# cqf7419/LiDAR-GS

Hardware: AMD Instinct MI355X
Metric: LiDAR range-view frames/sec (fwd+bwd) (higher is better)
Workload: dtype f32

## Files before the change

__graft_entry__.py:

```python
import os
import sys

ROOT = os.path.dirname(os.path.abspath(__file__))
for _p in (ROOT, os.path.join(ROOT, "lidar-gs_amd"), os.path.join(ROOT, "tests")):
    if _p not in sys.path:
        sys.path.insert(0, _p)


def build():
    import build_hip
    so = build_hip.build()
    assert os.path.exists(so), so
    from oracle import lgo
    lgo.build()
    import diff_lidargs_rasterization
    import lidargs_optim
    print("built:", so)
    print("built:", build_hip.OPTIM_OUT)


def smoke():
    import numpy as np
    import torch
    assert torch.cuda.is_available(), "smoke() needs a HIP device"
    import build_hip
    build_hip.build()
    import lidargs_scenes as sc
    from util import GRAD_KEYS_SR, hip_forward_backward, oracle_forward_backward, parity
    P, H, W, seed = 4000, 16, 512, 1
    scene = sc.make_scene("shell", P, H, seed, random_view=True)
    grads = sc.upstream_grads(H, W, seed)
    hip = hip_forward_backward(scene, W, H, grads, device="cuda:0")
    ref = oracle_forward_backward(scene, W, H, grads)
# ... 24 lines not shown
```

lidar-gs_amd/build_hip.py:

```python
import os
import subprocess
import sys
from concurrent.futures import ThreadPoolExecutor

HERE = os.path.dirname(os.path.abspath(__file__))
CSRC = os.path.join(HERE, "csrc")
OBJ = os.path.join(HERE, "build")
OUT = os.path.join(HERE, "diff_lidargs_rasterization", "liblidargs_hip.so")
COMMON = ["--offload-arch=gfx950", "-O3", "-std=c++17", "-fPIC", "-munsafe-fp-atomics", "-fno-gpu-rdc", "-Wall",
          "-Wno-unused-function", "-Wno-unused-value"]
SOURCES = {
    "api.hip": [],
    "preprocess.hip": ["-ffp-contract=off"],
    "binning.hip": [],
    "shard.hip": [],
    "render.hip": ["-fno-slp-vectorize"],
    "neural_gaussians.hip": [],
    "lidar_loss.hip": [],
    "chamfer.hip": ["-ffp-contract=off"],
    "surfel.hip": ["-ffp-contract=off", "-fno-slp-vectorize"],
    "anchor_growing.hip": ["-ffp-contract=off"],
    "knn.hip": ["-ffp-contract=off"],
    "metrics.hip": ["-ffp-contract=off"],
}
OPTIM_OUT = os.path.join(HERE, "lidargs_optim", "liblidargs_optim.so")
OPTIM_INCLUDE = os.path.join(HERE, "..", "include_optim")
OPTIM_SOURCES = {
    "adam.hip": ["-ffp-contract=off"],
}


def build_id():
    import hashlib
    h = hashlib.sha1()
    files = sorted(os.path.join(CSRC, f) for f in os.listdir(CSRC)) + sorted(
        os.path.join(HERE, "..", "include", f) for f in os.listdir(os.path.join(HERE, "..", "include"))) + sorted(
        os.path.join(OPTIM_INCLUDE, f) for f in os.listdir(OPTIM_INCLUDE)) + [os.path.abspath(__file__)]
    for f in files:
        h.update(os.path.basename(f).encode()); h.update(open(f, "rb").read())
    return h.hexdigest()[:12]


def box_id():
    try:
        import re
        out = subprocess.run(["rocm-smi", "--showuniqueid"], capture_output=True, text=True, timeout=20).stdout
        m = re.search(r"Unique ID:\s*(0x[0-9a-fA-F]+|\w+)", out)
        if m:
            return m.group(1)
    except Exception:
        pass
    return None


def _stale(out, deps):
    if not os.path.exists(out):
        return True
    t = os.path.getmtime(out)
    return any(os.path.getmtime(d) > t for d in deps)


def needs_build():
    return _stale(OUT, [os.path.join(CSRC, f) for f in os.listdir(CSRC) if f not in OPTIM_SOURCES]
                  + [os.path.join(HERE, "..", "include", "lidargs_rasterizer.h"), __file__])


def optim_needs_build():
    return _stale(OPTIM_OUT, [os.path.join(CSRC, f) for f in OPTIM_SOURCES]
                  + [os.path.join(OPTIM_INCLUDE, f) for f in os.listdir(OPTIM_INCLUDE)] + [__file__])


def build(force=False, verbose=False):
    if not force and not needs_build() and not optim_needs_build():
        return OUT
    import fcntl
    os.makedirs(OBJ, exist_ok=True)
    with open(os.path.join(OBJ, ".lock"), "w") as lock:
        fcntl.flock(lock, fcntl.LOCK_EX)
        try:
            if force or needs_build():
                _build_locked(SOURCES, OUT, verbose)
            if force or optim_needs_build():
                _build_locked(OPTIM_SOURCES, OPTIM_OUT, verbose)
            return OUT
        finally:
            fcntl.flock(lock, fcntl.LOCK_UN)


def _build_locked(sources, out, verbose):
    hipcc = os.environ.get("HIPCC", "/opt/rocm/bin/hipcc")
    extra_all = os.environ.get("LIDARGS_EXTRA_HIPCC_FLAGS", "").split()

    def compile_one(item):
        src, extra = item
        obj = os.path.join(OBJ, src.replace(".hip", ".o"))
        cmd = [hipcc] + COMMON + extra + extra_all + ["-c", os.path.join(CSRC, src), "-o", obj]
        if verbose:
            print(" ".join(cmd))
# ... 17 lines not shown
```

lidar-gs_amd/csrc/api.hip:

```cpp
#include "lidargs_common.h"
#include "../../include/lidargs_rasterizer.h"

#include <math.h>
#include <stdio.h>
#include <stdlib.h>
#include <string.h>
#include <limits>
#include <algorithm>
#include <mutex>

namespace {
using lg::SegPlan;

thread_local char g_err[512] = "";
thread_local long long g_counters[10] = {0, 0, 0, 0, 0, 0, 0, 0, -1, -1};
thread_local int g_counters_on = 0;
struct CounterPage {
    unsigned long long* dev = nullptr; unsigned long long* host = nullptr; hipEvent_t done = nullptr; int device = -1; bool pending = false;
    bool ready() {
        int d = -1;
        if (hipGetDevice(&d) != hipSuccess) return false;
        if (dev && d == device) return true;
        if (dev) { (void)hipFree(dev); dev = nullptr; }
        if (done) { (void)hipEventDestroy(done); done = nullptr; }
// ... 188 lines not shown
struct Profiler {
    static constexpr int MAX_CALLS = 256;
    struct Call { int n = 0; const char* names[LIDARGS_MAX_STAGES]; hipEvent_t ev[LIDARGS_MAX_STAGES + 1]; bool created = false; };
    bool enabled = false;
    int every = 1;
    int seen[2] = {0, 0};
    int ncalls = 0;
    Call* calls = nullptr;
    Call* cur = nullptr;
};
Profiler g_prof;
}

namespace lg {
int api_fail(int code, const char* msg) { return fail(code, "%s", msg); }
int api_check_launch(hipStream_t s, int debug, const char* what) { return check_launch(s, debug, what); }
int api_read_words_zero_behind(const uint32_t* dev, int n, uint32_t* out, void* zero, size_t zero_bytes, hipStream_t s) {
    hipError_t e = (hipError_t)read_words_begin(dev, n, s);
    if (e == hipSuccess && zero && zero_bytes) e = hipMemsetAsync(zero, 0, zero_bytes, s);
    return e == hipSuccess ? read_words_end(n, out) : (int)e;
}
bool prune_footprints() {
    static const bool on = [] { const char* e = getenv("LIDARGS_NO_PRUNE"); return !(e && atoi(e) != 0); }();
    return on;
}
int tile_rows() { return forced_tile_rows() ? forced_tile_rows() : 4; }

FrameLayout frame_layout(int num_rendered, int W, int H, int col_lo, int col_hi, FrameVariant variant) {
    const bool surfel = variant == FRAME_SURFEL, shell = variant == FRAME_SHELL;
    FrameLayout L;
// ... 285 lines not shown
    if (!geom_buffer || !binning_buffer || !image_buffer) return fail(LIDARGS_ERR_STATE, "backward: missing forward buffers%s");
    if (!means3D || !viewmatrix || !radii || !dL_dpix || !dL_dout_depth || !dL_dout_occ || !dL_dmean2D ||
        !dL_dopacity || !dL_dcolor || !dL_dmean3D || !dL_dscale || !dL_drot || (cov3D_precomp && !dL_dcov3D))
        return fail(LIDARGS_ERR_INVALID_ARGUMENT, "backward: NULL required pointer%s");

    lg::GeomView geom; lg::geom_carve(geom_buffer, (size_t)P, lg::GAUSS_BUFFERS, &geom);
    if (col_lo >= 0 && (col_lo % LG_TILE_W || col_hi <= col_lo || col_hi > width)) return fail(LIDARGS_ERR_INVALID_ARGUMENT, "backward: bad column wedge%s");
    const lg::FrameLayout L = lg::frame_layout(R, width, height, col_lo, col_hi, mode.is_shell ? lg::FRAME_SHELL : lg::FRAME_GAUSS);
    lg::BinView bin; L.bin_carve(binning_buffer, &bin);
    lg::ImgView img; lg::img_carve(image_buffer, width, height, lg::make_grid(width, height, 4).num_tiles(), &img);
    lg::prof_begin(stream, 1);

    lg::ZeroRows zr;
    zr.add(dL_dmean2D, 4); zr.add(dL_dconic, 4); zr.add(dL_dopacity, 1); zr.add(dL_dcolor, 2); zr.add(dL_ddepths, 1); zr.add(dL_dmean3D, 3);
    zr.add(dL_dsphere_means3D, 3); zr.add(dL_dbasis_u1, 3); zr.add(dL_dbasis_u2, 3); zr.add(dL_dcov3D, 6); zr.add(dL_dscale, 3); zr.add(dL_drot, 4);
    lg::launch_zero_touched(geom.touched, reinterpret_cast<float4*>(geom.gacc), 4, (size_t)P, geom.tlist, geom.tcount, zr, stream);
    lg::prof_mark("bwd_zero", stream);

    lg::RenderBwdArgs rb;
    rb.walk.cnt = nullptr;
    rb.grid = L.grid; rb.ranges = img.ranges; rb.point_list = bin.val_a; rb.rec = geom.rec; rb.rowspan = geom.rowspan;
    rb.coltab = img.coltab; rb.rowtab = img.rowtab; rb.bg = background; rb.final_T = img.final_T;
    rb.seg = bin.seg; rb.S = L.S; rb.seg_len = L.plan.seg_len;
    rb.alive = L.gated ? bin.alive : nullptr;
    rb.flags = L.flags ? bin.flags : nullptr; rb.R = L.Rp;
    rb.T_final_global = mode.T_final_global; rb.behind = mode.behind;
    rb.dL_dpix = dL_dpix; rb.dL_ddepth = dL_dout_depth; rb.dL_docc = dL_dout_occ; rb.gacc = geom.gacc;
    if (L.work_list) rb.walk = lg::work_list(bin);
    lg::launch_render_backward(rb, stream);
    LG_STAGE_CHECK("render backward");
    lg::prof_mark("render_bwd", stream);

    lg::GaussBwdArgs gb;
    gb.P = P; gb.scale_modifier = scale_modifier;
    gb.view = viewmatrix;
    gb.means3D = means3D; gb.scales = scales; gb.rotations = rotations; gb.cov3D_precomp = cov3D_precomp; gb.radii = radii;
    gb.gacc = geom.gacc; gb.tlist = geom.tlist; gb.tcount = geom.tcount;
    gb.dL_dmean2D = dL_dmean2D; gb.dL_dconic = dL_dconic; gb.dL_dopacity = dL_dopacity; gb.dL_dcolor = dL_dcolor;
    gb.dL_ddepths = dL_ddepths; gb.dL_dbasis_u1 = dL_dbasis_u1; gb.dL_dbasis_u2 = dL_dbasis_u2;
    gb.dL_dsphere = dL_dsphere_means3D; gb.dL_dmean3D = dL_dmean3D; gb.dL_dcov3D = dL_dcov3D; gb.dL_dscale = dL_dscale;
    gb.dL_drot = dL_drot;
    lg::launch_gaussian_backward(gb, stream);
    LG_STAGE_CHECK("gaussian backward");
// ... 448 lines not shown
```

lidar-gs_amd/csrc/lidargs_common.h:

```cpp
#pragma once
#include <hip/hip_runtime.h>
#include <stdint.h>
#include <stddef.h>

#define LG_TILE_W 16
#define LG_WAVE_ROWS 4
#define LG_CHANNELS 2

#define LG_SEG_TPASS 0
#define LG_SEG_C0 1
#define LG_SEG_C1 2
#define LG_SEG_D 3
#define LG_SEG_TEND 4
#define LG_SEG_TBREAK 5
#define LG_SEG_LAST 6
#define LG_SEG_PLANES 7

#define LG_REGION 256

namespace lg {

struct Carver {
    char* p;
    explicit Carver(char* base) : p(base) {}
// ... 238 lines not shown
    BufferWidths buf;
    size_t bin_carve(char* base, BinView* v) const { return lg::bin_carve(base, Rp, patches, grid.waves_per_tile, S, buf, v); }
};
FrameLayout frame_layout(int num_rendered, int W, int H, int col_lo, int col_hi, FrameVariant variant);

struct BinSpec {
    FrameVariant variant;
    int tile_rows;
    long long capacity;
    unsigned* status_host;
    const char* what;
};
struct BinnedFrame { FrameLayout L; BinView bin; size_t R; };
int bin_frame(const BinSpec& spec, const GeomView& geom, uint2* ranges, size_t P, int W, int H, int col_lo, int col_hi, bool compact,
              char* (*binning_alloc)(void*, size_t), void* binning_user, int debug, hipStream_t s, BinnedFrame* out);
struct ZeroRows { static constexpr int MAX = 12; float* p[MAX]; int w[MAX]; int n = 0;
                  void add(float* q, int width) { if (q && n < MAX) { p[n] = q; w[n] = width; n++; } } };
void launch_zero_touched(const uint8_t* touched, float4* acc, int line_f4, size_t P, uint8_t* tlist, uint16_t* tcount, const ZeroRows& zr, hipStream_t s);
void launch_touch_all(uint8_t* touched, const int* radii, size_t P, hipStream_t s);

void launch_setup_tables(const float* beams, int W, int H, ImgView img, hipStream_t s);
void launch_preprocess(const PreprocessParams& pp, const float* means3D, const float* scales, const float* rotations,
                       const float* opacities, const float* colors, const float* cov3D_precomp, const float* beams,
                       int* radii, int* radii_xy, GeomView g, const ImgView* tables, bool filter_only, hipStream_t s);
void launch_mark_visible(int P, const float* means3D, const float* view, unsigned char* present, hipStream_t s);
void launch_debug_rects(int n, int surfel, const float* p_cr, const int* r_xy, int gx, int gy, int* rects, hipStream_t s);

void launch_exclusive_scan(const uint32_t* in, uint32_t* out, size_t n, uint32_t* total_out, uint32_t* scratch, hipStream_t s);
struct RadixTail { const void* src = nullptr; void* dst = nullptr; int mode = 0; };
struct KeyBias { uint32_t kmin, cull; const uint32_t* lin_span = nullptr; };
struct RangeSortRest { KeyBias bias; int end_bit, max_bits; };
inline RangeSortRest range_sort_rest(uint32_t kinv, uint32_t kmax) {
    RangeSortRest r;
// ... 100 lines not shown

struct RenderBwdArgs {
    TileGrid grid;
    const uint2* ranges; const uint32_t* point_list; const float4* rec; const uint32_t* rowspan;
    const float2* coltab; const float2* rowtab;
    const float* bg;
    const float* final_T;
    const float* seg; int S; int seg_len;
    const uint8_t* flags; size_t R;
    const uint8_t* alive;
    const float* T_final_global;
    const float* behind;
    const float* dL_dpix; const float* dL_ddepth; const float* dL_docc;
    float* gacc;
    WorkList walk;
};
void launch_render_backward(const RenderBwdArgs& a, hipStream_t s);
void launch_count_backward_entries(const RenderBwdArgs& a, unsigned long long* out, hipStream_t s);
void note_forward(size_t P, size_t R, const FrameLayout& L, const uint32_t* totals, const uint8_t* flags, const uint8_t* touched,
                  const RenderBwdArgs* view, hipStream_t s);

struct GaussBwdArgs {
    int P; float scale_modifier; const float* view;
    const float* means3D; const float* scales; const float* rotations; const float* cov3D_precomp; const int* radii;
    const float* gacc;
    const uint8_t* tlist; const uint16_t* tcount;
    float* dL_dmean2D; float* dL_dconic; float* dL_dopacity; float* dL_dcolor; float* dL_ddepths;
    float* dL_dbasis_u1; float* dL_dbasis_u2;
    float* dL_dsphere; float* dL_dmean3D; float* dL_dcov3D; float* dL_dscale; float* dL_drot;
};
void launch_gaussian_backward(const GaussBwdArgs& a, hipStream_t s);
// ... 89 lines not shown
```

lidar-gs_amd/csrc/preprocess.hip:

```cpp
#include "lidargs_common.h"
#include "selection.h"
#include <algorithm>

namespace lg {

__device__ __forceinline__ float3 f3(float x, float y, float z) { return make_float3(x, y, z); }
__device__ __forceinline__ float dot3(float3 a, float3 b) { return a.x * b.x + a.y * b.y + a.z * b.z; }
__device__ __forceinline__ float3 scale3(float3 a, float s) { return f3(a.x * s, a.y * s, a.z * s); }
__device__ __forceinline__ float3 add3(float3 a, float3 b) { return f3(a.x + b.x, a.y + b.y, a.z + b.z); }

__device__ __forceinline__ float3 view_to_world(const float* vm, float3 v) {
    return f3(vm[0] * v.x + vm[1] * v.y + vm[2] * v.z,
              vm[4] * v.x + vm[5] * v.y + vm[6] * v.z,
              vm[8] * v.x + vm[9] * v.y + vm[10] * v.z);
}
__device__ __forceinline__ float3 world_to_view_dir(const float* vm, float3 v) {
    return f3(vm[0] * v.x + vm[4] * v.y + vm[8] * v.z,
              vm[1] * v.x + vm[5] * v.y + vm[9] * v.z,
              vm[2] * v.x + vm[6] * v.y + vm[10] * v.z);
}

struct Sym3 { float xx, xy, xz, yy, yz, zz; };
__device__ __forceinline__ float3 symmul(const Sym3& S, float3 v) {
    return f3(S.xx * v.x + S.xy * v.y + S.xz * v.z,
// ... 454 lines not shown

__global__ void __launch_bounds__(256) k_gaussian_backward(const GaussBwdArgs a) {
    const int lane = threadIdx.x & 63;
    const int region = blockIdx.x * 4 + (threadIdx.x >> 6);
    const int base = region * LG_REGION;
    if (base >= a.P) return;
    int off = (int)a.tlist[base + lane];
    int cnt = (int)a.tcount[region];
    asm volatile("" : "+v"(off), "+v"(cnt));
    for (int j = lane; j < cnt; j += 64) {
        gb_row(a, base + off);
        if (j + 64 < cnt) off = (int)a.tlist[base + j + 64];
    }
}

template <int LINE>
__global__ void __launch_bounds__(LG_REGION) k_zero_touched(const uint8_t* __restrict__ touched, float4* __restrict__ acc, size_t P,
                                                           uint8_t* __restrict__ tlist, uint16_t* __restrict__ tcount, const ZeroRows zr) {
    __shared__ uint32_t s_wcnt[LG_REGION / 64];
    const int tid = threadIdx.x, lane = tid & 63, wv = tid >> 6;
    const size_t base = (size_t)blockIdx.x * LG_REGION;
    const size_t i = base + tid;
    const bool mark = i < P && touched[i] != 0;
    const unsigned long long m0 = __ballot(mark);
    if (lane == 0) s_wcnt[wv] = (uint32_t)__popcll(m0);
    {
        unsigned long long m = m0;
        const size_t wbase = i - (size_t)lane;
        constexpr int PER = 64 / LINE;
        const int sub = lane / LINE, part = lane % LINE;
        const float4 z = make_float4(0.f, 0.f, 0.f, 0.f);
        while (m) {
            unsigned long long mm = m;
            int mine = -1;
#pragma unroll
            for (int k = 0; k < PER; k++) {
                const int j = mm ? __builtin_ctzll(mm) : -1;
                if (k == sub) mine = j;
                mm &= mm - 1ull;
            }
            m = mm;
            if (mine >= 0) acc[(wbase + (size_t)mine) * LINE + part] = z;
        }
    }
    if (i < P) {
        for (int k = 0; k < zr.n; k++) {
            float* q = zr.p[k];
            switch (zr.w[k]) {
                case 1: q[i] = 0.f; break;
                case 2: put2(q, i, 0.f, 0.f); break;
                case 3: put3(q, i, 0.f, 0.f, 0.f); break;
                case 4: put4(q, i, 0.f, 0.f, 0.f, 0.f); break;
                case 6: put3(q, 2 * i, 0.f, 0.f, 0.f); put3(q, 2 * i + 1, 0.f, 0.f, 0.f); break;
                default: for (int c = 0; c < zr.w[k]; c += 3) put3(q, (size_t)(zr.w[k] / 3) * i + c / 3, 0.f, 0.f, 0.f); break;
            }
        }
    }
    __syncthreads();
    uint32_t off = 0, total = 0;
#pragma unroll
    for (int v = 0; v < LG_REGION / 64; v++) { off += v < wv ? s_wcnt[v] : 0u; total += s_wcnt[v]; }
    if (mark) tlist[base + off + (uint32_t)__popcll(m0 & ((1ull << lane) - 1ull))] = (uint8_t)tid;
    if (tid == 0) tcount[blockIdx.x] = (uint16_t)total;
}
void launch_zero_touched(const uint8_t* touched, float4* acc, int line_f4, size_t P, uint8_t* tlist, uint16_t* tcount, const ZeroRows& zr, hipStream_t s) {
    const unsigned blocks = (unsigned)((P + LG_REGION - 1) / LG_REGION);
    if (!blocks) return;
    if (line_f4 == 8) hipLaunchKernelGGL(k_zero_touched<8>, dim3(blocks), dim3(LG_REGION), 0, s, touched, acc, P, tlist, tcount, zr);
    else hipLaunchKernelGGL(k_zero_touched<4>, dim3(blocks), dim3(LG_REGION), 0, s, touched, acc, P, tlist, tcount, zr);
}
__global__ void __launch_bounds__(256) k_touch_visible(uint8_t* __restrict__ touched, const int* __restrict__ radii, size_t P) {
    const size_t i = (size_t)blockIdx.x * 256 + threadIdx.x;
    if (i < P) touched[i] = radii[i] > 0 ? 1 : 0;
}
void launch_touch_all(uint8_t* touched, const int* radii, size_t P, hipStream_t s) {
    hipLaunchKernelGGL(k_touch_visible, dim3((unsigned)((P + 255) / 256)), dim3(256), 0, s, touched, radii, P);
}

void launch_gaussian_backward(const GaussBwdArgs& a, hipStream_t s) {
    const unsigned regions = (unsigned)((a.P + LG_REGION - 1) / LG_REGION);
    hipLaunchKernelGGL(k_gaussian_backward, dim3((regions + 3) / 4), dim3(256), 0, s, a);
}

}
// ... 1 lines not shown
```

lidar-gs_amd/csrc/render.hip:

```cpp
#include "lidargs_common.h"
#ifdef LG_PRECISE_EXP
#define LG_EXPF(x) expf(x)
#else
#define LG_EXPF(x) __expf(x)
#endif
#include <stdlib.h>

namespace lg {

#define LG_CHUNK 64

#ifdef LG_LANE_STATS
__device__ unsigned long long lg_lane_stats[16];
__device__ __forceinline__ void lane_stat(int base, unsigned long long m) {
    if (threadIdx.x % 64 == 0) {
        const int rows = ((m & 0xFFFFull) != 0) + ((m & 0xFFFF0000ull) != 0) + ((m & 0xFFFF00000000ull) != 0) + ((m >> 48) != 0);
        atomicAdd(&lg_lane_stats[base], 1ull); atomicAdd(&lg_lane_stats[base + 1], (unsigned long long)__popcll(m));
        atomicAdd(&lg_lane_stats[base + 2], (unsigned long long)rows); atomicAdd(&lg_lane_stats[base + 3], m ? 1ull : 0ull);
    }
}
void lane_stats_read(unsigned long long* out, int reset) {
    (void)hipMemcpyFromSymbol(out, HIP_SYMBOL(lg_lane_stats), sizeof(unsigned long long) * 16);
    if (reset) { unsigned long long z[16] = {0}; (void)hipMemcpyToSymbol(HIP_SYMBOL(lg_lane_stats), z, sizeof z); }
}
// ... 788 lines not shown
            const float keep = hi ? v[k + 2] : v[k], send = hi ? v[k] : v[k + 2];
            v[k] = keep + xchg_xor1(send);
        }
    }
    {
        const bool hi = lane & 2;
        const float keep = hi ? v[1] : v[0], send = hi ? v[0] : v[1];
        v[0] = keep + xchg_xor2(send);
    }
    v[0] += __int_as_float(__builtin_amdgcn_update_dpp(0, __float_as_int(v[0]), 0x124, 0xF, 0xF, true));
    v[0] += __int_as_float(__builtin_amdgcn_update_dpp(0, __float_as_int(v[0]), 0x128, 0xF, 0xF, true));
    return v[0];
}

template <bool V2>
#ifdef LG_BWD_WAVES
__attribute__((amdgpu_waves_per_eu(LG_BWD_WAVES, LG_BWD_WAVES)))
#endif
__global__ void __launch_bounds__(64) k_render_backward(const RenderBwdArgs a) {
    constexpr int OFS = V2 ? 2 : 0;
    __shared__ float4 s_rec_[4 * (LG_CHUNK + OFS)];
    __shared__ float4 s_oprow_[LG_CHUNK + OFS];
    __shared__ uint32_t s_gid_[LG_CHUNK + OFS];
    constexpr int CS = LG_CHUNK + OFS;
    float4* const s_rec = s_rec_ + OFS;
    float4* const s_oprow = s_oprow_ + OFS;
    uint32_t* const s_gid = s_gid_ + OFS;
    const int lane = threadIdx.x;
    const int S = a.S;
    const int wpt = a.grid.waves_per_tile;
    int patch, seg;
    if (a.walk.cnt) {
        const unsigned r = blockIdx.x % LG_WORK_REGIONS, i = blockIdx.x / LG_WORK_REGIONS;
        if (i >= a.walk.cnt[r * LG_WORK_CNT_STRIDE]) return;
// ... 182 lines not shown
            int jb = ja;
            if (more_b) jb = top(todo);
            rb = read(jb);
            evaluate(ra, ja);
            if (!more_b) break;
            const bool more_a = todo != 0ull;
            ja = jb;
            if (more_a) ja = top(todo);
            ra = read(ja);
            evaluate(rb, jb);
            if (!more_a) break;
        }
    }
}

__global__ void __launch_bounds__(64) k_count_backward_entries(const RenderBwdArgs a, unsigned long long* __restrict__ out) {
    const int lane = threadIdx.x;
    const int S = a.S, wpt = a.grid.waves_per_tile;
    int patch, seg;
    if (!block_patch_segment(blockIdx.x, a.grid.window_patches(), S, patch, seg)) return;
    patch = a.grid.global_patch(patch);
    const int tile = patch / wpt, sub = patch - tile * wpt;
    const size_t stride = LG_SEG_PLANES * 64;
    const uint2 tr = a.ranges[tile];
    const int St = segment_count(tr, S, a.seg_len);
    const int limit = a.alive ? (int)a.alive[patch] : 255;
    if (seg >= St || seg >= limit) return;
    uint32_t n_max = reinterpret_cast<const uint32_t*>(a.seg + (size_t)patch * S * stride + lane)[(size_t)seg * stride + LG_SEG_LAST * 64];
#pragma unroll
    for (int o = 32; o > 0; o >>= 1) n_max = max(n_max, (uint32_t)__shfl_xor((int)n_max, o));
    if (n_max == 0) return;
    const uint2 sr = segment_range(tr, St, seg);
    const uint8_t* fl = a.flags ? a.flags + (size_t)sub * a.R + sr.x : nullptr;
    uint32_t c = 0;
    for (uint32_t k = lane; k < n_max; k += 64) c += (!fl || fl[k] != 0) ? 1u : 0u;
#pragma unroll
    for (int o = 32; o > 0; o >>= 1) c += __shfl_xor(c, o);
    if (lane == 0 && c) atomicAdd(out, (unsigned long long)c);
}
void launch_count_backward_entries(const RenderBwdArgs& a, unsigned long long* out, hipStream_t s) {
    hipLaunchKernelGGL(k_count_backward_entries, dim3(segment_grid(a.grid.window_patches(), a.S)), dim3(64), 0, s, a, out);
}

void launch_render_backward(const RenderBwdArgs& a, hipStream_t s) {
    const unsigned blocks = a.walk.cnt ? (unsigned)LG_WORK_REGIONS * a.walk.cap : segment_grid(a.grid.window_patches(), a.S);
    if (walk2() & 4) hipLaunchKernelGGL(k_render_backward<true>, dim3(blocks), dim3(64), 0, s, a);
    else hipLaunchKernelGGL(k_render_backward<false>, dim3(blocks), dim3(64), 0, s, a);
}

}
```

lidar-gs_amd/csrc/surfel.hip:

```cpp
#include "lidargs_common.h"
#include <string.h>

namespace lg {

#define SF_CHUNK 64
typedef float sf2 __attribute__((ext_vector_type(2)));
#define SF_NEAR_N 0.2f
#define SF_FAR_N 80.0f

__device__ __forceinline__ float3 sf3(float x, float y, float z) { return make_float3(x, y, z); }
__device__ __forceinline__ float sdot(float3 a, float3 b) { return a.x * b.x + a.y * b.y + a.z * b.z; }

__device__ __forceinline__ bool sf_pix(float3 p, int W, int H, const float* __restrict__ beams, bool with_cull, float col_step, float2& pix) {
    const float pi_f = 3.14159265358979323846f;
    const float p_c = (pi_f - (float)atan2((double)p.y, (double)p.x)) / col_step;
    const float alpha = (float)atan2((double)p.z, (double)sqrtf(p.x * p.x + p.y * p.y));
    int bi;
    if (alpha >= beams[H - 1]) bi = H - 1;
    else if (alpha <= beams[0]) bi = 0;
    else {
        int lo = 0, hi = H;
        while (lo < hi) { const int md = (lo + hi) >> 1; if (beams[md] < alpha) lo = md + 1; else hi = md; }
        bi = lo;
    }
// ... 635 lines not shown

enum { SFA_COL0 = 0, SFA_COL1 = 1, SFA_OPA = 2, SFA_N0 = 4, SFA_N1 = 5, SFA_N2 = 6, SFA_TU0 = 8, SFA_TU1 = 9, SFA_TU2 = 10,
       SFA_TV0 = 12, SFA_TV1 = 13, SFA_TV2 = 16, SFA_TW0 = 17, SFA_TW1 = 18, SFA_TW2 = 20, SFA_AW0 = 21, SFA_AW1 = 22, SFA_AW2 = 24,
       SFA_M2X = 25, SFA_M2Y = 26, SFA_M2AX = 28, SFA_M2AY = 29, SFA_Z2D = 30 };

struct SfBwdArgs {
    TileGrid grid;
    const uint2* ranges; const uint32_t* point_list; const float4* rec; const uint32_t* rowspan;
    const float2* coltab; const float2* rowtab; const float* bg;
    const float* accum; const uint32_t* n_contrib;
    const float* dL_dpix; const float* dL_dothers;
    float* gacc;
    const float* seg; int S; int seg_len;
    const uint8_t* flags; size_t R;
    const uint8_t* alive;
};

#ifdef LG_SF_BWD_WAVES
__attribute__((amdgpu_waves_per_eu(LG_SF_BWD_WAVES, LG_SF_BWD_WAVES)))
#endif
__global__ void __launch_bounds__(64) k_sf_render_backward(const SfBwdArgs a) {
    __shared__ float4 s_rec[5 * SF_CHUNK];
    __shared__ float4 s_oprow[SF_CHUNK];
    __shared__ uint32_t s_gid[SF_CHUNK];
    const int lane = threadIdx.x;
    const int S = a.S;
    const int wpt = a.grid.waves_per_tile;
    int patch, seg;
    if (!block_patch_segment(blockIdx.x, a.grid.num_tiles() * wpt, S, patch, seg)) return;
    const int tile = patch / wpt, sub = patch - tile * wpt;
    const uint2 tr = a.ranges[tile];
    const int St = segment_count(tr, S, a.seg_len);
    if (seg >= St) return;
    if (a.alive && seg >= (int)a.alive[patch]) return;
    const size_t stride = SF_SEG_PLANES * 64;
    const float* sb = a.seg + (size_t)patch * S * stride + lane;
// ... 131 lines not shown
            v[SFA_AW0] = fabsf(gTw.x); v[SFA_AW1] = fabsf(gTw.y); v[SFA_AW2] = fabsf(gTw.z);
            v[SFA_M2X] = m2x; v[SFA_M2Y] = m2y; v[SFA_M2AX] = fabsf(m2x); v[SFA_M2AY] = fabsf(m2y);
            v[SFA_Z2D] = in3d ? 0.f : dL_dz;
            T = Tn;
            acc_c0 = a_c0; acc_d = a_d; acc_a = a_a; acc_n0 = a_n0; acc_n1 = a_n1; acc_n2 = a_n2;
            l_c0 = r1.w; l_d = c_d; l_n0 = r3.x; l_n1 = r3.y; l_n2 = r3.z;
            last_alpha = alpha;
            const float mine = sf_reduce_scatter32(v, lane);
            if ((lane & 8) == 0) {
                const int slot = 16 * ((lane >> 5) & 1) + 8 * ((lane >> 4) & 1) + 4 * (lane & 1) + 2 * ((lane >> 1) & 1) + ((lane >> 2) & 1);
                if (!((SFA_DEAD >> slot) & 1u)) atomicAdd(a.gacc + 32 * (size_t)s_gid[j] + slot, mine);
            }
        }
    }
}

void launch_sf_render_backward(const SfBwdArgs& a, hipStream_t s) {
    hipLaunchKernelGGL(k_sf_render_backward, dim3(segment_grid(a.grid.num_tiles() * a.grid.waves_per_tile, a.S)), dim3(64), 0, s, a);
}

struct SfGaussBwdArgs {
    int P, W, H;
    const float* view; const float* means3D; const float* scales; const float* rotations; const float* beams; const int* radii;
    const float* transMat;
    const float* gacc; const uint8_t* tlist; const uint16_t* tcount;
    float* dL_dmean2D; float* dL_dnormal; float* dL_dopacity; float* dL_dcolor; float* dL_dmean3D; float* dL_dtransMat;
    float* dL_dtransMat_2dtemp; float* dL_dscale; float* dL_drot; float* depth;
};

__device__ __forceinline__ void sf_gb_row(const SfGaussBwdArgs& a, const int idx);
__global__ void __launch_bounds__(256) k_sf_gaussian_backward(const SfGaussBwdArgs a) {
    const int lane = threadIdx.x & 63;
    {
// ... 106 lines not shown
```

lidar-gs_amd/csrc/surfel_api.inc:

```
#include "../../include/lidargs_rasterizer.h"
#include <math.h>

namespace lg {

static_assert(SURFEL_BUFFERS.seg_planes == SF_SEG_PLANES, "lidargs_common.h SURFEL_BUFFERS carves the surfel blend's segment planes");
struct SfImgView { float* accum; uint32_t* n_contrib; uint2* ranges; float2* coltab; float2* rowtab; };
static size_t sf_img_carve(char* base, int W, int H, int tiles, SfImgView* v) {
    Carver c(base);
    SfImgView m;
    const size_t N = (size_t)W * H;
    m.accum = c.take<float>(3 * N); m.n_contrib = c.take<uint32_t>(2 * N); m.ranges = c.take<uint2>(tiles);
    m.coltab = c.take<float2>(W); m.rowtab = c.take<float2>(H);
    if (v) *v = m;
    return (size_t)(c.p - base) + 128;
}

}

#define SF_CHECK(what) do { int rc_ = lg::api_check_launch(stream, debug, what); if (rc_) return rc_; } while (0)
#define SF_HIP(call) do { hipError_t e_ = (call); if (e_ != hipSuccess) return lg::api_fail(LIDARGS_ERR_HIP, hipGetErrorString(e_)); } while (0)

extern "C" {

int lidargs_surfel_forward(lidargs_alloc_fn geometry_alloc, void* geometry_user, lidargs_alloc_fn binning_alloc, void* binning_user,
// ... 93 lines not shown
    hipStream_t stream = (hipStream_t)stream_;
    if (P < 0 || R < 0 || width <= 0 || height < 2) return lg::api_fail(LIDARGS_ERR_INVALID_ARGUMENT, "surfel backward: bad sizes");
    if (P == 0) return 0;
    if (!geom_buffer || !binning_buffer || !image_buffer) return lg::api_fail(LIDARGS_ERR_STATE, "surfel backward: missing forward buffers");
    if (!means3D || !scales || !rotations || !viewmatrix || !beam_inclinations || !background || !radii || !dL_dpix || !dL_depths || !dL_dmean2D ||
        !dL_dopacity || !dL_dcolor || !dL_dmean3D || !dL_dscale || !dL_drot || !depth)
        return lg::api_fail(LIDARGS_ERR_INVALID_ARGUMENT, "surfel backward: NULL required pointer");
    const lg::FrameLayout L = lg::frame_layout(R, width, height, -1, -1, lg::FRAME_SURFEL);
    lg::GeomView geom; lg::geom_carve(geom_buffer, (size_t)P, lg::SURFEL_BUFFERS, &geom);
    lg::BinView bin; L.bin_carve(binning_buffer, &bin);
    lg::SfImgView img; lg::sf_img_carve(image_buffer, width, height, L.grid.num_tiles(), &img);
    lg::prof_begin(stream, 1);
    lg::ZeroRows zr;
    zr.add(dL_dmean2D, 4); zr.add(dL_dnormal, 3); zr.add(dL_dopacity, 1); zr.add(dL_dcolor, 2); zr.add(dL_dmean3D, 3); zr.add(dL_dtransMat, 9);
    zr.add(dL_dtransMat_2dtemp, 3); zr.add(dL_dscale, 2); zr.add(dL_drot, 4);
    lg::launch_zero_touched(geom.touched, reinterpret_cast<float4*>(geom.gacc), 8, (size_t)P, geom.tlist, geom.tcount, zr, stream);
    lg::prof_mark("bwd_zero", stream);
    lg::SfBwdArgs ba;
    ba.grid = L.grid; ba.ranges = img.ranges; ba.point_list = bin.val_a; ba.rec = geom.rec; ba.rowspan = geom.rowspan;
    ba.coltab = img.coltab; ba.rowtab = img.rowtab; ba.bg = background; ba.accum = img.accum; ba.n_contrib = img.n_contrib;
    ba.dL_dpix = dL_dpix; ba.dL_dothers = dL_depths; ba.gacc = geom.gacc;
    ba.seg = bin.seg; ba.S = L.S; ba.seg_len = L.plan.seg_len; ba.flags = bin.flags; ba.R = L.Rp;
    ba.alive = L.gated ? bin.alive : nullptr;
    lg::launch_sf_render_backward(ba, stream);
    SF_CHECK("surfel render backward");
    lg::prof_mark("render_bwd", stream);
    lg::SfGaussBwdArgs ga;
    ga.P = P; ga.W = width; ga.H = height; ga.view = viewmatrix; ga.means3D = means3D; ga.scales = scales; ga.rotations = rotations;
    ga.beams = beam_inclinations; ga.radii = radii; ga.transMat = transMat_precomp; ga.gacc = geom.gacc; ga.tlist = geom.tlist; ga.tcount = geom.tcount;
    ga.dL_dmean2D = dL_dmean2D; ga.dL_dnormal = dL_dnormal; ga.dL_dopacity = dL_dopacity; ga.dL_dcolor = dL_dcolor; ga.dL_dmean3D = dL_dmean3D;
    ga.dL_dtransMat = dL_dtransMat; ga.dL_dtransMat_2dtemp = dL_dtransMat_2dtemp; ga.dL_dscale = dL_dscale; ga.dL_drot = dL_drot; ga.depth = depth;
    lg::launch_sf_gaussian_backward(ga, stream);
    SF_CHECK("surfel gaussian backward");
    lg::prof_mark("gaussian_bwd", stream);
    return 0;
}

int lidargs_surfel_visible_filter(lidargs_alloc_fn geometry_alloc, void* geometry_user, lidargs_alloc_fn binning_alloc, void* binning_user,
// ... 25 lines not shown
```

Measured before the change: 1462.

## Fuse gradient-row zeroing into render backward kernel tail

Moves the zeroing of per-Gaussian output gradient arrays from the zero_touched kernel into the tail of the render backward kernel. Each block clears a contiguous 16-byte-aligned share of the merged arrays after its blend walk. The choice is made by a per-block byte threshold or the LIDARGS_BLEND_ZERO environment variable. The intent is to hide the memset traffic in the backward kernel's idle or tail time. The cost is extra work and a larger kernel argument struct on every backward block, plus a new debug library for testing the fill.

```diff
diff --git a/__graft_entry__.py b/__graft_entry__.py
--- a/__graft_entry__.py
+++ b/__graft_entry__.py
@@ -17,6 +17,8 @@
     import lidargs_optim
     print("built:", so)
     print("built:", build_hip.OPTIM_OUT)
+    assert os.path.exists(build_hip.DEBUG_OUT), build_hip.DEBUG_OUT
+    print("built:", build_hip.DEBUG_OUT)
 
 
 def smoke():
diff --git a/include_debug/lidargs_debug.h b/include_debug/lidargs_debug.h
--- /dev/null
+++ b/include_debug/lidargs_debug.h
@@ -0,0 +1,16 @@
+#ifndef LIDARGS_DEBUG_H
+#define LIDARGS_DEBUG_H
+#include <stddef.h>
+#ifdef __cplusplus
+extern "C" {
+#endif
+
+#define LIDARGS_DEBUG_ABI_VERSION 1
+int lidargs_debug_abi_version(void);
+
+int lidargs_debug_zero_rows(int n, float* const* arrays, const int* widths, size_t P, size_t blocks, void* stream);
+
+#ifdef __cplusplus
+}
+#endif
+#endif
diff --git a/lidar-gs_amd/build_hip.py b/lidar-gs_amd/build_hip.py
--- a/lidar-gs_amd/build_hip.py
+++ b/lidar-gs_amd/build_hip.py
@@ -28,6 +28,11 @@
 OPTIM_SOURCES = {
     "adam.hip": ["-ffp-contract=off"],
 }
+DEBUG_OUT = os.path.join(HERE, "diff_lidargs_rasterization", "liblidargs_debug.so")
+DEBUG_INCLUDE = os.path.join(HERE, "..", "include_debug")
+DEBUG_SOURCES = {
+    "zero_rows_debug.hip": [],
+}
 
 
 def build_id():
@@ -35,7 +40,8 @@
     h = hashlib.sha1()
     files = sorted(os.path.join(CSRC, f) for f in os.listdir(CSRC)) + sorted(
         os.path.join(HERE, "..", "include", f) for f in os.listdir(os.path.join(HERE, "..", "include"))) + sorted(
-        os.path.join(OPTIM_INCLUDE, f) for f in os.listdir(OPTIM_INCLUDE)) + [os.path.abspath(__file__)]
+        os.path.join(OPTIM_INCLUDE, f) for f in os.listdir(OPTIM_INCLUDE)) + sorted(
+        os.path.join(DEBUG_INCLUDE, f) for f in os.listdir(DEBUG_INCLUDE)) + [os.path.abspath(__file__)]
     for f in files:
         h.update(os.path.basename(f).encode()); h.update(open(f, "rb").read())
     return h.hexdigest()[:12]
@@ -61,7 +67,7 @@
 
 
 def needs_build():
-    return _stale(OUT, [os.path.join(CSRC, f) for f in os.listdir(CSRC) if f not in OPTIM_SOURCES]
+    return _stale(OUT, [os.path.join(CSRC, f) for f in os.listdir(CSRC) if f not in OPTIM_SOURCES and f not in DEBUG_SOURCES]
                   + [os.path.join(HERE, "..", "include", "lidargs_rasterizer.h"), __file__])
 
 
@@ -70,8 +76,13 @@
                   + [os.path.join(OPTIM_INCLUDE, f) for f in os.listdir(OPTIM_INCLUDE)] + [__file__])
 
 
+def debug_needs_build():
+    return _stale(DEBUG_OUT, [os.path.join(CSRC, f) for f in DEBUG_SOURCES] + [os.path.join(CSRC, "lidargs_common.h")]
+                  + [os.path.join(DEBUG_INCLUDE, f) for f in os.listdir(DEBUG_INCLUDE)] + [__file__])
+
+
 def build(force=False, verbose=False):
-    if not force and not needs_build() and not optim_needs_build():
+    if not force and not needs_build() and not optim_needs_build() and not debug_needs_build():
         return OUT
     import fcntl
     os.makedirs(OBJ, exist_ok=True)
@@ -82,6 +93,8 @@
                 _build_locked(SOURCES, OUT, verbose)
             if force or optim_needs_build():
                 _build_locked(OPTIM_SOURCES, OPTIM_OUT, verbose)
+            if force or debug_needs_build():
+                _build_locked(DEBUG_SOURCES, DEBUG_OUT, verbose)
             return OUT
         finally:
             fcntl.flock(lock, fcntl.LOCK_UN)
diff --git a/lidar-gs_amd/csrc/api.hip b/lidar-gs_amd/csrc/api.hip
--- a/lidar-gs_amd/csrc/api.hip
+++ b/lidar-gs_amd/csrc/api.hip
@@ -226,6 +226,14 @@
 
 namespace lg {
 int api_fail(int code, const char* msg) { return fail(code, "%s", msg); }
+
+constexpr size_t BLEND_FILL_MAX = 16384;
+bool blend_takes_fill(size_t fill_bytes, unsigned blend_blocks) {
+    static const int env = [] { const char* e = getenv("LIDARGS_BLEND_ZERO"); return e ? (atoi(e) != 0 ? 1 : 0) : -1; }();
+    if (!fill_bytes || !blend_blocks) return false;
+    if (env >= 0) return env != 0;
+    return (fill_bytes + blend_blocks - 1) / blend_blocks <= BLEND_FILL_MAX;
+}
 int api_check_launch(hipStream_t s, int debug, const char* what) { return check_launch(s, debug, what); }
 int api_read_words_zero_behind(const uint32_t* dev, int n, uint32_t* out, void* zero, size_t zero_bytes, hipStream_t s) {
     hipError_t e = (hipError_t)read_words_begin(dev, n, s);
@@ -541,8 +549,6 @@
     lg::ZeroRows zr;
     zr.add(dL_dmean2D, 4); zr.add(dL_dconic, 4); zr.add(dL_dopacity, 1); zr.add(dL_dcolor, 2); zr.add(dL_ddepths, 1); zr.add(dL_dmean3D, 3);
     zr.add(dL_dsphere_means3D, 3); zr.add(dL_dbasis_u1, 3); zr.add(dL_dbasis_u2, 3); zr.add(dL_dcov3D, 6); zr.add(dL_dscale, 3); zr.add(dL_drot, 4);
-    lg::launch_zero_touched(geom.touched, reinterpret_cast<float4*>(geom.gacc), 4, (size_t)P, geom.tlist, geom.tcount, zr, stream);
-    lg::prof_mark("bwd_zero", stream);
 
     lg::RenderBwdArgs rb;
     rb.walk.cnt = nullptr;
@@ -554,6 +560,10 @@
     rb.T_final_global = mode.T_final_global; rb.behind = mode.behind;
     rb.dL_dpix = dL_dpix; rb.dL_ddepth = dL_dout_depth; rb.dL_docc = dL_dout_occ; rb.gacc = geom.gacc;
     if (L.work_list) rb.walk = lg::work_list(bin);
+    const bool blend_fills = lg::blend_takes_fill(zr.bytes((size_t)P), lg::render_backward_blocks(rb));
+    lg::launch_zero_touched(geom.touched, reinterpret_cast<float4*>(geom.gacc), 4, (size_t)P, geom.tlist, geom.tcount, zr, !blend_fills, stream);
+    lg::prof_mark("bwd_zero", stream);
+    if (blend_fills) { zr.plan((size_t)P); rb.zero = zr; rb.zero_P = (size_t)P; }
     lg::launch_render_backward(rb, stream);
     LG_STAGE_CHECK("render backward");
     lg::prof_mark("render_bwd", stream);
diff --git a/lidar-gs_amd/csrc/lidargs_common.h b/lidar-gs_amd/csrc/lidargs_common.h
--- a/lidar-gs_amd/csrc/lidargs_common.h
+++ b/lidar-gs_amd/csrc/lidargs_common.h
@@ -276,9 +276,60 @@
 struct BinnedFrame { FrameLayout L; BinView bin; size_t R; };
 int bin_frame(const BinSpec& spec, const GeomView& geom, uint2* ranges, size_t P, int W, int H, int col_lo, int col_hi, bool compact,
               char* (*binning_alloc)(void*, size_t), void* binning_user, int debug, hipStream_t s, BinnedFrame* out);
-struct ZeroRows { static constexpr int MAX = 12; float* p[MAX]; int w[MAX]; int n = 0;
-                  void add(float* q, int width) { if (q && n < MAX) { p[n] = q; w[n] = width; n++; } } };
-void launch_zero_touched(const uint8_t* touched, float4* acc, int line_f4, size_t P, uint8_t* tlist, uint16_t* tcount, const ZeroRows& zr, hipStream_t s);
+struct ZeroRows {
+    static constexpr int MAX = 12;
+    float* p[MAX]; int w[MAX]; int n = 0;
+    float* rp[MAX]; int rw[MAX]; int nr = 0;
+    unsigned long long roff[MAX], vtotal = 0, share = 0;
+    void add(float* q, int width) { if (q && n < MAX) { p[n] = q; w[n] = width; n++; } }
+    size_t bytes(size_t P) const { size_t b = 0; for (int k = 0; k < n; k++) b += 4 * P * (size_t)w[k]; return b; }
+    static __host__ __device__ unsigned long long slots(uintptr_t beg, uintptr_t end) { return beg < end ? ((end + 15) >> 4) - (beg >> 4) : 0ull; }
+    void plan(size_t P) {
+        int ord[MAX];
+        for (int k = 0; k < n; k++) { int j = k; for (; j > 0 && p[ord[j - 1]] > p[k]; j--) ord[j] = ord[j - 1]; ord[j] = k; }
+        nr = 0; vtotal = 0;
+        for (int i = 0; i < n && P; i++) {
+            const int k = ord[i];
+            if (nr && rp[nr - 1] + P * (size_t)rw[nr - 1] == p[k]) rw[nr - 1] += w[k];
+            else { rp[nr] = p[k]; rw[nr] = w[k]; nr++; }
+        }
+        for (int k = 0; k < nr; k++) {
+            const uintptr_t beg = (uintptr_t)rp[k];
+            vtotal += ((beg >> 4) - vtotal) & 7ull;
+            roff[k] = vtotal;
+            vtotal += slots(beg, beg + 4 * P * (size_t)rw[k]);
+        }
+    }
+    static unsigned long long share_of(unsigned long long vtotal, unsigned long long G) { return G ? ((vtotal + G - 1) / G + 7ull) & ~7ull : 0ull; }
+    void cut(unsigned G) { share = share_of(vtotal, G); }
+};
+__host__ __device__ inline void zero_rows_share(unsigned long long vtotal, unsigned long long share, unsigned b, unsigned long long& lo, unsigned long long& hi) {
+    lo = (unsigned long long)b * share; if (lo > vtotal) lo = vtotal;
+    hi = lo + share; if (hi > vtotal) hi = vtotal;
+}
+#ifdef __HIPCC__
+__device__ __forceinline__ void zero_rows_fill(const ZeroRows& zr, size_t P, unsigned b) {
+    unsigned long long lo, hi;
+    zero_rows_share(zr.vtotal, zr.share, b, lo, hi);
+    if (lo >= hi) return;
+    const float4 z = make_float4(0.f, 0.f, 0.f, 0.f);
+    for (int k = 0; k < zr.nr; k++) {
+        const uintptr_t beg = (uintptr_t)zr.rp[k], end = beg + 4 * P * (size_t)zr.rw[k];
+        const unsigned long long v0 = zr.roff[k], v1 = v0 + ZeroRows::slots(beg, end);
+        const unsigned long long s0 = lo > v0 ? lo : v0, s1 = hi < v1 ? hi : v1;
+        for (unsigned long long s = s0 + threadIdx.x; s < s1; s += blockDim.x) {
+            const uintptr_t at = (beg & ~(uintptr_t)15) + 16 * (s - v0);
+            if (at >= beg && at + 16 <= end) *reinterpret_cast<float4*>(at) = z;
+            else {
+#pragma unroll
+                for (int c = 0; c < 4; c++) if (at + 4 * c >= beg && at + 4 * c < end) *reinterpret_cast<float*>(at + 4 * c) = 0.f;
+            }
+        }
+    }
+}
+#endif
+bool blend_takes_fill(size_t fill_bytes, unsigned blend_blocks);
+void launch_zero_touched(const uint8_t* touched, float4* acc, int line_f4, size_t P, uint8_t* tlist, uint16_t* tcount, const ZeroRows& zr, bool rows, hipStream_t s);
 void launch_touch_all(uint8_t* touched, const int* radii, size_t P, hipStream_t s);
 
 void launch_setup_tables(const float* beams, int W, int H, ImgView img, hipStream_t s);
@@ -409,7 +460,9 @@
     const float* dL_dpix; const float* dL_ddepth; const float* dL_docc;
     float* gacc;
     WorkList walk;
-};
+    ZeroRows zero; size_t zero_P = 0;
+};
+unsigned render_backward_blocks(const RenderBwdArgs& a);
 void launch_render_backward(const RenderBwdArgs& a, hipStream_t s);
 void launch_count_backward_entries(const RenderBwdArgs& a, unsigned long long* out, hipStream_t s);
 void note_forward(size_t P, size_t R, const FrameLayout& L, const uint32_t* totals, const uint8_t* flags, const uint8_t* touched,
diff --git a/lidar-gs_amd/csrc/preprocess.hip b/lidar-gs_amd/csrc/preprocess.hip
--- a/lidar-gs_amd/csrc/preprocess.hip
+++ b/lidar-gs_amd/csrc/preprocess.hip
@@ -492,7 +492,7 @@
     }
 }
 
-template <int LINE>
+template <int LINE, bool ROWS>
 __global__ void __launch_bounds__(LG_REGION) k_zero_touched(const uint8_t* __restrict__ touched, float4* __restrict__ acc, size_t P,
                                                            uint8_t* __restrict__ tlist, uint16_t* __restrict__ tcount, const ZeroRows zr) {
     __shared__ uint32_t s_wcnt[LG_REGION / 64];
@@ -521,7 +521,7 @@
             if (mine >= 0) acc[(wbase + (size_t)mine) * LINE + part] = z;
         }
     }
-    if (i < P) {
+    if (ROWS && i < P) {
         for (int k = 0; k < zr.n; k++) {
             float* q = zr.p[k];
             switch (zr.w[k]) {
@@ -541,11 +541,11 @@
     if (mark) tlist[base + off + (uint32_t)__popcll(m0 & ((1ull << lane) - 1ull))] = (uint8_t)tid;
     if (tid == 0) tcount[blockIdx.x] = (uint16_t)total;
 }
-void launch_zero_touched(const uint8_t* touched, float4* acc, int line_f4, size_t P, uint8_t* tlist, uint16_t* tcount, const ZeroRows& zr, hipStream_t s) {
+void launch_zero_touched(const uint8_t* touched, float4* acc, int line_f4, size_t P, uint8_t* tlist, uint16_t* tcount, const ZeroRows& zr, bool rows, hipStream_t s) {
     const unsigned blocks = (unsigned)((P + LG_REGION - 1) / LG_REGION);
     if (!blocks) return;
-    if (line_f4 == 8) hipLaunchKernelGGL(k_zero_touched<8>, dim3(blocks), dim3(LG_REGION), 0, s, touched, acc, P, tlist, tcount, zr);
-    else hipLaunchKernelGGL(k_zero_touched<4>, dim3(blocks), dim3(LG_REGION), 0, s, touched, acc, P, tlist, tcount, zr);
+    auto k = line_f4 == 8 ? (rows ? k_zero_touched<8, true> : k_zero_touched<8, false>) : (rows ? k_zero_touched<4, true> : k_zero_touched<4, false>);
+    hipLaunchKernelGGL(k, dim3(blocks), dim3(LG_REGION), 0, s, touched, acc, P, tlist, tcount, zr);
 }
 __global__ void __launch_bounds__(256) k_touch_visible(uint8_t* __restrict__ touched, const int* __restrict__ radii, size_t P) {
     const size_t i = (size_t)blockIdx.x * 256 + threadIdx.x;
diff --git a/lidar-gs_amd/csrc/render.hip b/lidar-gs_amd/csrc/render.hip
--- a/lidar-gs_amd/csrc/render.hip
+++ b/lidar-gs_amd/csrc/render.hip
@@ -826,10 +826,7 @@
 }
 
 template <bool V2>
-#ifdef LG_BWD_WAVES
-__attribute__((amdgpu_waves_per_eu(LG_BWD_WAVES, LG_BWD_WAVES)))
-#endif
-__global__ void __launch_bounds__(64) k_render_backward(const RenderBwdArgs a) {
+__device__ __forceinline__ void render_backward_walk(const RenderBwdArgs& a) {
     constexpr int OFS = V2 ? 2 : 0;
     __shared__ float4 s_rec_[4 * (LG_CHUNK + OFS)];
     __shared__ float4 s_oprow_[LG_CHUNK + OFS];
@@ -1042,6 +1039,15 @@
     }
 }
 
+template <bool V2>
+#ifdef LG_BWD_WAVES
+__attribute__((amdgpu_waves_per_eu(LG_BWD_WAVES, LG_BWD_WAVES)))
+#endif
+__global__ void __launch_bounds__(64) k_render_backward(const RenderBwdArgs a) {
+    render_backward_walk<V2>(a);
+    if (a.zero.nr) zero_rows_fill(a.zero, a.zero_P, blockIdx.x);
+}
+
 __global__ void __launch_bounds__(64) k_count_backward_entries(const RenderBwdArgs a, unsigned long long* __restrict__ out) {
     const int lane = threadIdx.x;
     const int S = a.S, wpt = a.grid.waves_per_tile;
@@ -1070,8 +1076,13 @@
     hipLaunchKernelGGL(k_count_backward_entries, dim3(segment_grid(a.grid.window_patches(), a.S)), dim3(64), 0, s, a, out);
 }
 
-void launch_render_backward(const RenderBwdArgs& a, hipStream_t s) {
-    const unsigned blocks = a.walk.cnt ? (unsigned)LG_WORK_REGIONS * a.walk.cap : segment_grid(a.grid.window_patches(), a.S);
+unsigned render_backward_blocks(const RenderBwdArgs& a) {
+    return a.walk.cnt ? (unsigned)LG_WORK_REGIONS * a.walk.cap : segment_grid(a.grid.window_patches(), a.S);
+}
+void launch_render_backward(const RenderBwdArgs& a_, hipStream_t s) {
+    RenderBwdArgs a = a_;
+    const unsigned blocks = render_backward_blocks(a);
+    a.zero.cut(blocks);
     if (walk2() & 4) hipLaunchKernelGGL(k_render_backward<true>, dim3(blocks), dim3(64), 0, s, a);
     else hipLaunchKernelGGL(k_render_backward<false>, dim3(blocks), dim3(64), 0, s, a);
 }
diff --git a/lidar-gs_amd/csrc/surfel.hip b/lidar-gs_amd/csrc/surfel.hip
--- a/lidar-gs_amd/csrc/surfel.hip
+++ b/lidar-gs_amd/csrc/surfel.hip
@@ -673,12 +673,10 @@
     const float* seg; int S; int seg_len;
     const uint8_t* flags; size_t R;
     const uint8_t* alive;
+    ZeroRows zero; size_t zero_P = 0;
 };
 
-#ifdef LG_SF_BWD_WAVES
-__attribute__((amdgpu_waves_per_eu(LG_SF_BWD_WAVES, LG_SF_BWD_WAVES)))
-#endif
-__global__ void __launch_bounds__(64) k_sf_render_backward(const SfBwdArgs a) {
+__device__ __forceinline__ void sf_render_backward_walk(const SfBwdArgs& a) {
     __shared__ float4 s_rec[5 * SF_CHUNK];
     __shared__ float4 s_oprow[SF_CHUNK];
     __shared__ uint32_t s_gid[SF_CHUNK];
@@ -840,9 +838,20 @@
         }
     }
 }
-
-void launch_sf_render_backward(const SfBwdArgs& a, hipStream_t s) {
-    hipLaunchKernelGGL(k_sf_render_backward, dim3(segment_grid(a.grid.num_tiles() * a.grid.waves_per_tile, a.S)), dim3(64), 0, s, a);
+#ifdef LG_SF_BWD_WAVES
+__attribute__((amdgpu_waves_per_eu(LG_SF_BWD_WAVES, LG_SF_BWD_WAVES)))
+#endif
+__global__ void __launch_bounds__(64) k_sf_render_backward(const SfBwdArgs a) {
+    sf_render_backward_walk(a);
+    if (a.zero.nr) zero_rows_fill(a.zero, a.zero_P, blockIdx.x);
+}
+
+unsigned sf_render_backward_blocks(const SfBwdArgs& a) { return segment_grid(a.grid.num_tiles() * a.grid.waves_per_tile, a.S); }
+void launch_sf_render_backward(const SfBwdArgs& a_, hipStream_t s) {
+    SfBwdArgs a = a_;
+    const unsigned blocks = sf_render_backward_blocks(a);
+    a.zero.cut(blocks);
+    hipLaunchKernelGGL(k_sf_render_backward, dim3(blocks), dim3(64), 0, s, a);
 }
 
 struct SfGaussBwdArgs {
diff --git a/lidar-gs_amd/csrc/surfel_api.inc b/lidar-gs_amd/csrc/surfel_api.inc
--- a/lidar-gs_amd/csrc/surfel_api.inc
+++ b/lidar-gs_amd/csrc/surfel_api.inc
@@ -131,14 +131,16 @@
     lg::ZeroRows zr;
     zr.add(dL_dmean2D, 4); zr.add(dL_dnormal, 3); zr.add(dL_dopacity, 1); zr.add(dL_dcolor, 2); zr.add(dL_dmean3D, 3); zr.add(dL_dtransMat, 9);
     zr.add(dL_dtransMat_2dtemp, 3); zr.add(dL_dscale, 2); zr.add(dL_drot, 4);
-    lg::launch_zero_touched(geom.touched, reinterpret_cast<float4*>(geom.gacc), 8, (size_t)P, geom.tlist, geom.tcount, zr, stream);
-    lg::prof_mark("bwd_zero", stream);
     lg::SfBwdArgs ba;
     ba.grid = L.grid; ba.ranges = img.ranges; ba.point_list = bin.val_a; ba.rec = geom.rec; ba.rowspan = geom.rowspan;
     ba.coltab = img.coltab; ba.rowtab = img.rowtab; ba.bg = background; ba.accum = img.accum; ba.n_contrib = img.n_contrib;
     ba.dL_dpix = dL_dpix; ba.dL_dothers = dL_depths; ba.gacc = geom.gacc;
     ba.seg = bin.seg; ba.S = L.S; ba.seg_len = L.plan.seg_len; ba.flags = bin.flags; ba.R = L.Rp;
     ba.alive = L.gated ? bin.alive : nullptr;
+    const bool blend_fills = lg::blend_takes_fill(zr.bytes((size_t)P), lg::sf_render_backward_blocks(ba));
+    lg::launch_zero_touched(geom.touched, reinterpret_cast<float4*>(geom.gacc), 8, (size_t)P, geom.tlist, geom.tcount, zr, !blend_fills, stream);
+    lg::prof_mark("bwd_zero", stream);
+    if (blend_fills) { zr.plan((size_t)P); ba.zero = zr; ba.zero_P = (size_t)P; }
     lg::launch_sf_render_backward(ba, stream);
     SF_CHECK("surfel render backward");
     lg::prof_mark("render_bwd", stream);
diff --git a/lidar-gs_amd/csrc/zero_rows_debug.hip b/lidar-gs_amd/csrc/zero_rows_debug.hip
--- /dev/null
+++ b/lidar-gs_amd/csrc/zero_rows_debug.hip
@@ -0,0 +1,26 @@
+#include "lidargs_common.h"
+#include "../../include_debug/lidargs_debug.h"
+
+namespace {
+__global__ void __launch_bounds__(64) k_debug_zero_rows(const lg::ZeroRows zr, size_t P) { lg::zero_rows_fill(zr, P, blockIdx.x); }
+}
+
+extern "C" {
+
+int lidargs_debug_abi_version(void) { return LIDARGS_DEBUG_ABI_VERSION; }
+
+int lidargs_debug_zero_rows(int n, float* const* arrays, const int* widths, size_t P, size_t blocks, void* stream) {
+    if (n < 0 || n > lg::ZeroRows::MAX || blocks == 0 || blocks > 0x7FFFFFFFull) return -1;
+    if (n && (!arrays || !widths)) return -1;
+    lg::ZeroRows zr;
+    for (int k = 0; k < n; k++) {
+        if (!arrays[k] || ((uintptr_t)arrays[k] & 3) || widths[k] < 1 || widths[k] > 9) return -1;
+        zr.add(arrays[k], widths[k]);
+    }
+    zr.plan(P);
+    zr.cut((unsigned)blocks);
+    hipLaunchKernelGGL(k_debug_zero_rows, dim3((unsigned)blocks), dim3(64), 0, (hipStream_t)stream, zr, P);
+    return hipGetLastError() == hipSuccess ? 0 : -2;
+}
+
+}
```

Result: slower. 1445 (-1.1%).
